# rssalessio/TZDDPC

Measured on NVIDIA B200. Metric: closed-loop TZDDPC steps/sec over batched scenarios, higher is better.
Workload: dtype f64

## Files before the change

### tzddpc_b200/csrc/tz_admm.cuh

```cuda
#pragma once
#include "tz_common.cuh"

namespace tz {

#ifndef TZ_SPO_MIN
#define TZ_SPO_MIN 16
#endif
template <int NZ_, int N2_, int NU_, int NL_, int G_, int NPAR_, int NAG_, int NCHK_, int MINB_>
struct Bucket {
  static constexpr int NZ = NZ_, N2 = N2_, NU = NU_, NL = NL_, G = G_, NPAR = NPAR_, NAG = NAG_, NCHK = NCHK_;
  static constexpr int MINB = MINB_;
  static constexpr int NCL = N2 + NU + NL;
  static constexpr int NC = NCL * G;
  static constexpr int NK = N2 * G;
  static constexpr int NCOL = 1 + 2 * NPAR + NAG;
  static constexpr int NCHL = (NCHK + G - 1) / G;
  static constexpr int TPB = 128;
  static constexpr int WPB = TPB / 32;
  static constexpr int SPW = 32 / G;
  static constexpr int TPO = (SPW >= TZ_SPO_MIN) ? 1 : TZ_SPO_MIN / SPW;
  static constexpr int SPO = SPW * TPO;
  static constexpr int HP = NPAR / 2;
  static constexpr int OM_V = 1, OM_P = 1 + NZ, NW = 1 + NZ + NPAR;
  static constexpr int OM_C = NW, OM_XP = NW + HP, KOM = NW + 2 * HP;
  static constexpr int PRE_ROWS = 4 * HP + G;
  static constexpr int NCOL2 = (NCOL + 1) / 2;
  static constexpr int NCOLP = 2 * NCOL2 + ((2 * NCOL2) % 8 == 0 ? 2 : 0);
  static_assert(NCL <= 32 && (G & (G - 1)) == 0 && G <= 32 && N2 >= 1 && NAG >= 1, "bad bucket");
};

template <class BK>
struct QpProg {
  double P[BK::NZ][BK::NZ];
  double A[BK::NC][BK::NZ];
  double l0[BK::NC], u0[BK::NC];
  double kink0[BK::NK], wabs[BK::NK];
  double R[BK::NC][BK::NCOLP];
  double Rs[BK::NC];
  double q0[BK::NZ];
  double Qp[BK::NZ][BK::NPAR];
  double Bt[BK::NAG][BK::NPAR];
  double gam[BK::NAG];
  double Rchk[BK::NCHK][BK::NCOLP];
  double chk_tol[BK::NCHK];
  double cc[BK::NCOL];
  double CC2[BK::NPAR][BK::NPAR];
  double D[BK::NZ];
  double Einv[BK::NC];
  double sing_inv[BK::NC];
  double cinv;
  int sing_var[BK::NC];
  int row_of_slot[BK::NC];
  int grp_order[BK::NC];
  int grp_new[BK::NC];
  double grp_sgn[BK::NC];
  int grp_first[BK::NC + 4];
  int ngrp;
// ... 671 lines not shown
```

### tzddpc_b200/csrc/tz_fast.cuh

```cuda
#pragma once
#include <cstdlib>

#include "tz_step.cuh"

namespace tz {

constexpr int kDeferTile = TZ_SPO_MIN;

constexpr int fast_ctas_per_sm(int tpb) { return tpb >= 512 ? 1 : 512 / tpb; }

template <class BK, int TPB, int NSLOT, int H = 1, bool PL = false>
__global__ void __launch_bounds__(TPB * H, fast_ctas_per_sm(TPB * H))
    fast_step_kernel(const QpProg<BK>* __restrict__ gpg, const Aux ax, const SolverParams sp, const StepArgs a,
                     const SetEntry* __restrict__ entries, const int32_t* __restrict__ tile_prog, const int slot_bytes) {
  constexpr int NZ = BK::NZ, NPAR = BK::NPAR, HP = BK::NPAR / 2, NCOL = BK::NCOL, NW = BK::NW, G = BK::G;
  static_assert(kDeferTile == 16 && BK::SPO == 16, "deferred tiles are the 16-scenario output tiles of step_kernel");
  static_assert(NSLOT <= 1 || TPB == 32, "two program slots: one warp per CTA");
  constexpr int OM_X = NW + HP, OM_NS = NW + 2 * HP;
  constexpr int QPB = (int)((sizeof(QpProg<BK>) + 15) & ~(size_t)15);
  extern __shared__ __align__(16) unsigned char smem_raw[];
  const int tix = threadIdx.x, tid = tix % TPB, hq = tix / TPB, lane = tix & 31;
  constexpr int NT = TPB * H;
  const int n = ax.n, m = ax.m, nv = ax.nv;
  const bool closed = a.x != nullptr;
  const int64_t LD = a.ld;
  const bool dense = a.ze1 != nullptr && !sp.tube_packed;
  double (*om)[TPB] = reinterpret_cast<double (*)[TPB]>(smem_raw + (NSLOT > 1 ? NSLOT : 1) * (size_t)slot_bytes);
  int* sflag = reinterpret_cast<int*>(&om[NW + 3 * HP][0]);
  const int n_tab = H > 1 ? ax.o_zrow : ax.n_dbl;
  auto stage = [&](unsigned char* slot, const void* pg_src, const double* tab_src) {
    const char* src = reinterpret_cast<const char*>(pg_src);
    char* dst = reinterpret_cast<char*>(slot);
    double* td = reinterpret_cast<double*>(slot + QPB);
    constexpr int NCH = (int)(sizeof(QpProg<BK>) / 16);
    for (int i = tix; i < NCH; i += NT) cp_async16(dst + 16 * i, src + 16 * i);
    if (tix == 0 && (sizeof(QpProg<BK>) % 16) != 0) cp_async8(dst + 16 * NCH, src + 16 * NCH);
    for (int i = tix; i < n_tab; i += NT) cp_async8(td + i, tab_src + i);
  };
  auto stage_plant = [&](unsigned char* slot) {
    double* td = reinterpret_cast<double*>(slot + QPB);
    if (closed && !PL) {
      for (int i = tix; i < n * n; i += NT) cp_async8(td + n_tab + i, a.A_true + i);
      for (int i = tix; i < n * m; i += NT) cp_async8(td + n_tab + n * n + i, a.B_true + i);
    }
  };
  pdl_trigger();
  unsigned char* my_slot = smem_raw;
  if constexpr (NSLOT == 0) {
    stage(smem_raw, gpg, ax.tab);
  } else {
    constexpr int TILES = TPB / kDeferTile;
    const int64_t last_tile = (a.S + kDeferTile - 1) / kDeferTile - 1;
    const int64_t t0 = (int64_t)blockIdx.x * TILES;
    const int j0 = tile_prog[t0 < last_tile ? t0 : last_tile];
    stage(smem_raw, entries[j0].pg, entries[j0].tab);
    if constexpr (NSLOT == 2) {
      const int j1 = tile_prog[t0 + 1 < last_tile ? t0 + 1 : last_tile];
      if (j1 != j0) {
        stage(smem_raw + slot_bytes, entries[j1].pg, entries[j1].tab);
        if (lane >= 16) my_slot = smem_raw + slot_bytes;
      }
    }
  }
  cp_async_commit();
  pdl_wait();
  stage_plant(smem_raw);
  if constexpr (NSLOT == 2) stage_plant(smem_raw + slot_bytes);
  cp_async_commit();
  double* tabd = reinterpret_cast<double*>(my_slot + QPB);
  bool staged = false;
  const QpProg<BK>& pg = *reinterpret_cast<const QpProg<BK>*>(my_slot);
  const double* sXB = tabd + ax.o_XB;
  const double* sCZ = tabd + ax.o_CZ;
  const double* sK = tabd + ax.o_K;
  const double* sA = tabd + n_tab;
  const double* sB = sA + n * n;
  const double2* tt = reinterpret_cast<const double2*>(tabd + ax.o_tt);
  const int* zs = reinterpret_cast<const int*>(tabd + ax.o_zrun);
  const bool zvec = dense && (reinterpret_cast<uintptr_t>(a.ze1) & 15u) == 0 && (a.ld & 1) == 0 && (a.S & 1) == 0 &&
                    (int64_t)(ax.n * (1 + ax.g1)) * a.ld * 8 < (int64_t)0x7fffffff;
  const int* zrow = reinterpret_cast<const int*>(tabd + ax.o_zrow);
  const int64_t nblk = (a.S + TPB - 1) / TPB;
  const unsigned long long* hint = reinterpret_cast<const unsigned long long*>(a.warm);
  unsigned long long* hint_w = reinterpret_cast<unsigned long long*>(a.warm);
  const unsigned half_mask = lane < 16 ? 0x0000ffffu : 0xffff0000u;
  const double* omc = &om[0][tid];

  for (int64_t blk = blockIdx.x; blk < nblk; blk += (NSLOT == 0 ? (int64_t)gridDim.x : nblk)) {
    const int64_t s = blk * TPB + tid;
    const bool live = s < a.S;
    const int64_t sc = live ? s : a.S - 1;
    bool emit = false, good = false;
    enum { kDefer = -2 };
    int status = kDefer;
    double omr[NW];
    double nrm2 = 0.0, cost = NAN;
    auto zero_runs = [&]() {
      double* base = a.ze1 + s;
#pragma unroll 1
      for (int r = 0; r < ax.n_zrun; ++r) {
        double* ptr = base + (int64_t)zs[2 * r] * LD;
#pragma unroll 4
        for (int c = zs[2 * r + 1]; c > 0; --c, ptr += LD) __stcs(ptr, 0.0);
      }
    };
    constexpr int CPR = TPB / 2;
    const int z_half = tid / CPR;
    const int64_t z_sv = blk * TPB + 2 * (tid % CPR);
    int z_pos = z_half * ax.n_zrow_half;
    const int z_stop = z_pos + ax.n_zrow_half;
    if (!(zvec && z_sv < a.S) || H > 1) z_pos = z_stop;
    char* const z_base = reinterpret_cast<char*>(a.ze1 + z_sv);
    const int ld8 = (int)(LD * 8);
    auto drip = [&](int budget) {
      int k = z_stop - z_pos;
      k = k < budget ? k : budget;
#pragma unroll 2
      for (; k > 0; k -= 4, z_pos += 4) {
        const int4 r = *reinterpret_cast<const int4*>(zrow + z_pos);
        const double2 z2 = make_double2(0.0, 0.0);
        __stcs(reinterpret_cast<double2*>(z_base + (int64_t)r.x * ld8), z2);
        __stcs(reinterpret_cast<double2*>(z_base + (int64_t)r.y * ld8), z2);
        __stcs(reinterpret_cast<double2*>(z_base + (int64_t)r.z * ld8), z2);
        __stcs(reinterpret_cast<double2*>(z_base + (int64_t)r.w * ld8), z2);
      }
    };
    const bool zero_first = H == 1 && dense && !zvec && (((tid >> 5) + (int)blk) & 1);
    if (hq == 0) {
    double w[2 * BK::NCOL2];
// ... 70 lines not shown
    if (__any_sync(0xffffffffu, status == kDefer && valid)) {
      const bool inf = singleton_infeasible2<BK>(pg, w);
      if (status == kDefer && valid && inf) status = TZ_STATUS_INFEASIBLE;
    }
    const unsigned dmask = __ballot_sync(0xffffffffu, live && status == kDefer);
    const bool deferred = (dmask & half_mask) != 0u;
    if (deferred && (lane & 15) == 0 && live) {
      const int slot = atomicAdd(a.defer, 1);
      if (slot >= 0 && slot < (a.S + kDeferTile - 1) / kDeferTile) a.defer_list[slot] = (int32_t)(s / kDeferTile);
    }
    emit = live && !deferred;
    good = status == TZ_STATUS_OK;
    drip(16);
    if (emit) {
#pragma unroll
      for (int g = 0; g < G; ++g) {
        unsigned long long wnext = 0ull;
        if (good) {
          wnext = code[g] | kCodeValid;
          if (fresh) hint_w[(int64_t)(G + g) * LD + s] = wnext;
        } else if (a.x_restart != nullptr) {
          const unsigned long long h0 = hint[(int64_t)(G + g) * LD + s];
          wnext = (h0 & kCodeValid) ? (h0 | kCodeFresh) : 0ull;
        }
        hint_w[(int64_t)g * LD + s] = wnext;
      }
      omr[0] = 1.0;
#pragma unroll
      for (int j = 0; j < NZ; ++j) omr[BK::OM_V + j] = (j < nv) ? (good ? pg.D[j] * res.x[j] : NAN) : 0.0;
#pragma unroll
      for (int j = 0; j < NPAR; ++j) omr[BK::OM_P + j] = w[1 + j];
      if (good) cost = fma(res.obj, pg.cinv, c0);
      else if (status == TZ_STATUS_INFEASIBLE) cost = INFINITY;
#pragma unroll
      for (int j = 0; j < NW; ++j) om[j][tid] = omr[j];
#pragma unroll 2
      for (int r = 0; r < n; ++r) {
        const double* row = sCZ + r * NW;
        double acc = 0.0;
#pragma unroll
        for (int j = 0; j < NW; ++j) acc = fma(row[j], omr[j], acc);
        om[BK::OM_C + r][tid] = acc;
      }
      drip(16);
    }
    if constexpr (H > 1) sflag[tid] = (emit ? 1 : 0) | (good ? 2 : 0);
    } else {
      if (!staged) {
        cp_async_wait<0>();
        __syncthreads();
        staged = true;
      }
      if (dense && live) {
        double* base = a.ze1 + s;
#pragma unroll 1
        for (int r = hq - 1; r < ax.n_zrun; r += H - 1) {
          double* ptr = base + (int64_t)zs[2 * r] * LD;
#pragma unroll 4
          for (int c = zs[2 * r + 1]; c > 0; --c, ptr += LD) __stcs(ptr, 0.0);
        }
      }
    }
    if constexpr (H > 1) {
      __syncthreads();
      if (hq > 0) {
        const int f = sflag[tid];
        emit = (f & 1) != 0;
        good = (f & 2) != 0;
        if (emit) {
#pragma unroll
          for (int j = 0; j < NW; ++j) omr[j] = omc[j * TPB];
        }
      }
    }
    if (emit) {
      if (a.ze1 != nullptr) {
        double* base = a.ze1 + s;
        if (sp.tube_packed) {
          double* ptr = base + (int64_t)hq * LD;
#pragma unroll 4
          for (int i = hq; i < ax.n_nz; i += H, ptr += H * LD) {
            const double2 e = tt[i];
            __stcs(ptr, e.x * omc[(int)(__double_as_longlong(e.y) & 0xffffffffll) * TPB]);
          }
        } else {
          if constexpr (H == 1) {
            if (!zero_first && !zvec) zero_runs();
          }
#pragma unroll 4
          for (int i = hq; i < ax.n_nz; i += H) {
            const double2 e = tt[i];
            const long long ie = __double_as_longlong(e.y);
            __stcs(base + (ie >> 32) * LD, e.x * omc[(int)(ie & 0xffffffffll) * TPB]);
          }
        }
      }
      double xb1[HP];
#pragma unroll
      for (int i = 0; i < HP; ++i) xb1[i] = 0.0;
      auto xb_row = [&](int i) {
        const double* row = sXB + i * NW;
        double acc = 0.0;
#pragma unroll
        for (int j = 0; j < NW; ++j) acc = fma(row[j], omr[j], acc);
        if (a.xbar_traj != nullptr) a.xbar_traj[(int64_t)i * LD + s] = acc;
        return acc;
      };
      if constexpr (H == 1) {
        if (a.xbar_traj != nullptr) {
#pragma unroll 2
          for (int i = 0; i < n; ++i) (void)xb_row(i);
        }
        drip(16);
        if (a.xbar_traj != nullptr || closed) {
#pragma unroll
          for (int k = 0; k < HP; ++k)
            if (k < n) xb1[k] = xb_row(n + k);
        }
        drip(16);
        if (a.xbar_traj != nullptr) {
#pragma unroll 2
          for (int i = 2 * n; i < (ax.N + 1) * n; ++i) (void)xb_row(i);
        }
      } else {
        if (hq == 0 && (a.xbar_traj != nullptr || closed)) {
#pragma unroll
          for (int k = 0; k < HP; ++k)
            if (k < n) xb1[k] = xb_row(n + k);
        }
        if (a.xbar_traj != nullptr && hq > 0) {
#pragma unroll 1
          for (int i = hq - 1; i < (ax.N + 1) * n; i += H - 1)
            if (i < n || i >= 2 * n) (void)xb_row(i);
        }
      }
      if (hq == 0) {
      if (a.v != nullptr)
        for (int j = 0; j < nv; ++j) a.v[(int64_t)j * LD + s] = omc[(BK::OM_V + j) * TPB];
      if (a.status) a.status[s] = status;
      if (a.iters) a.iters[s] = 0;
      if (a.cost) a.cost[s] = cost;
      if (closed) {
        double us[kMaxM];
#pragma unroll
        for (int j = 0; j < kMaxM; ++j) {
          double acc = 0.0;
          if (j < m) {
            acc = omr[BK::OM_V + (j < NZ ? j : 0)];
#pragma unroll
            for (int i = 0; i < HP; ++i)
              if (i < n) acc = fma(sK[j * n + i], omr[BK::OM_P + HP + i], acc);
            if (a.u_out) a.u_out[(int64_t)j * LD + s] = good ? acc : NAN;
          }
          us[j] = acc;
        }
        double xo[HP];
        cp_async_wait<0>();
#pragma unroll
        for (int i = 0; i < HP; ++i) xo[i] = (i < n) ? omc[(OM_X + i) * TPB] : 0.0;
#pragma unroll
        for (int i = 0; i < HP; ++i) {
          if (i < n) {
            double acc = a.noise ? omc[(OM_NS + i) * TPB] : 0.0;
            if constexpr (PL) {
              const double* ab = a.AB_true + (int64_t)i * (n + m) * LD + s;
#pragma unroll
              for (int k = 0; k < HP; ++k)
                if (k < n) acc = fma(ab[(int64_t)k * LD], xo[k], acc);
#pragma unroll
              for (int k = 0; k < kMaxM; ++k)
                if (k < m) acc = fma(ab[(int64_t)(n + k) * LD], us[k], acc);
// ... 135 lines not shown
```

### tzddpc_b200/csrc/tz_fused.cu

```cuda
#include "tz_step.cuh"
#include "tz_big.h"

namespace tz {

template <class BK>
int launch_fast(const TzProgram* p, const SolverParams& sp, const StepArgs& a, cudaStream_t st);
extern template int launch_fast<B0>(const TzProgram*, const SolverParams&, const StepArgs&, cudaStream_t);
template <class BK>
int launch_fast_set(const TzProgram* p0, const SolverParams& sp, const StepArgs& a, const SetEntry* entries, const int32_t* tile_prog,
                    int block, cudaStream_t st);
extern template int launch_fast_set<B0>(const TzProgram*, const SolverParams&, const StepArgs&, const SetEntry*, const int32_t*, int,
                                        cudaStream_t);
extern template int launch_bucket<B1>(const TzProgram*, const SolverParams&, const StepArgs&, cudaStream_t);
extern template int launch_bucket<B2>(const TzProgram*, const SolverParams&, const StepArgs&, cudaStream_t);
extern template int launch_bucket<B3>(const TzProgram*, const SolverParams&, const StepArgs&, cudaStream_t);
extern template int launch_bucket_set<B1>(const TzProgram*, const SetEntry*, int, int64_t, const SolverParams&, const StepArgs&, cudaStream_t);
extern template int launch_bucket_set<B2>(const TzProgram*, const SetEntry*, int, int64_t, const SolverParams&, const StepArgs&, cudaStream_t);
extern template int launch_bucket_set<B3>(const TzProgram*, const SetEntry*, int, int64_t, const SolverParams&, const StepArgs&, cudaStream_t);
extern template int launch_bucket_set_run<B1>(const TzProgram*, const SetEntry*, int, int64_t, const SolverParams&, const StepArgs&, cudaStream_t);
extern template int launch_bucket_set_run<B2>(const TzProgram*, const SetEntry*, int, int64_t, const SolverParams&, const StepArgs&, cudaStream_t);
extern template int launch_bucket_set_run<B3>(const TzProgram*, const SetEntry*, int, int64_t, const SolverParams&, const StepArgs&, cudaStream_t);

constexpr int64_t kHotMinBatch = 256;

struct RowClasses { int n2 = 0, nu = 0, nl = 0; };

static RowClasses classify(const TzProgramDesc& d, std::vector<int>* cls) {
  RowClasses rc;
  for (int i = 0; i < d.nc; ++i) {
    const bool lf = std::isfinite(d.l0[i]), uf = std::isfinite(d.u0[i]);
    int c = 0;
    if (d.wabs[i] > 0.0 || (lf && uf) || (!lf && !uf)) c = 0;
// ... 113 lines not shown
      g.grp_first[gi++] = t;
      for (size_t k = 0; k < mem.size(); ++k, ++t) {
        g.grp_order[t] = mem[k].first;
        g.grp_new[t] = k == 0 ? 1 : 0;
        g.grp_sgn[t] = mem[k].second;
      }
    }
    g.ngrp = gi;
    for (; gi < BK::NC + 4; ++gi) g.grp_first[gi] = t;
    for (; t < BK::NC; ++t) { g.grp_order[t] = 0; g.grp_new[t] = 0; g.grp_sgn[t] = 1.0; }
  }
  g.cinv = 1.0 / d.c;
  g.nz = nz; g.nc = nc; g.npar = npar; g.nag = nag; g.nchk = d.nchk;
  g.has_cc2 = 0;
  for (int a = 0; a < npar * npar; ++a) g.has_cc2 |= (d.CC2[a] != 0.0) ? 1 : 0;
}

}

using namespace tz;

struct HostImage {
  std::vector<unsigned char> packed, aux;
};

template <class BK>
static int create_bucket(const TzProgramDesc& d, TzProgram* p, int id, HostImage& img) {
  p->bucket = id;
  img.packed.assign(sizeof(QpProg<BK>), 0);
  pack<BK>(d, *reinterpret_cast<QpProg<BK>*>(img.packed.data()));
  p->NZ = BK::NZ;
  p->NC = BK::NC;
  p->G = BK::G;
  p->NW = BK::NW; p->OM_V = BK::OM_V; p->OM_P = BK::OM_P; p->OM_C = BK::OM_C; p->HP = BK::NPAR / 2;
  return TZ_OK;
}

static int use_big_path(const TzProgramDesc* d, TzProgram* p) {
  p->bucket = 4;
  p->NZ = d->nz; p->NC = d->nc; p->G = 32;
  p->nz = d->nz; p->nc = d->nc; p->n = d->n; p->m = d->m; p->N = d->horizon; p->nv = d->nv; p->g1 = d->g1; p->npar = d->npar;
  for (int e = 0; e < d->n * (1 + d->g1); ++e)
    if (d->ze1_ptr[e + 1] > d->ze1_ptr[e]) p->tube_ent.push_back(e);
  p->aux.n_nz = (int)p->tube_ent.size();
  p->aux.n = d->n; p->aux.m = d->m; p->aux.N = d->horizon; p->aux.nv = d->nv; p->aux.g1 = d->g1;
  return TZ_OK;
}

static int build_program_host(const TzProgramDesc* d, TzProgram* p, HostImage& img) {
  TZ_REQUIRE(d != nullptr, "null argument");
  TZ_REQUIRE(d->n >= 1 && d->n <= kMaxN && d->m >= 1 && d->m <= kMaxM, "dim_x must be 1..%d and dim_u 1..%d", kMaxN, kMaxM);
  TZ_REQUIRE(d->npar == 2 * d->n, "npar must be 2*dim_x");
  TZ_REQUIRE(d->nv == d->horizon * d->m && d->nv <= 16 && d->nz >= d->nv, "bad nv/nz");
  TZ_REQUIRE(d->nc >= 0 && d->na >= 0 && d->nchk >= 0 && d->g1 >= 0 && d->nterms >= 0 && d->nkink >= 0 && d->nkink <= d->nc,
             "negative size in the program descriptor");
  TZ_REQUIRE(d->ze1_ptr && d->ze1_ptr[0] == 0, "ze1_ptr[0] must be 0");
  for (int e = 0; e < d->n * (1 + d->g1); ++e)
    TZ_REQUIRE(d->ze1_ptr[e + 1] >= d->ze1_ptr[e], "ze1_ptr must be non-decreasing (entry %d)", e);
  TZ_REQUIRE(d->ze1_ptr[d->n * (1 + d->g1)] == d->nterms, "ze1_ptr[n(1+g1)] must equal nterms");
  int rc = TZ_ERANGE;
#define TZ_TRY(BK, ID) \
  if (rc == TZ_ERANGE && fits<BK>(*d)) rc = create_bucket<BK>(*d, p, ID, img);
  TZ_TRY(B0, 0) TZ_TRY(B1, 1) TZ_TRY(B2, 2) TZ_TRY(B3, 3)
#undef TZ_TRY
  if (rc == TZ_ERANGE && big_fits(*d)) return use_big_path(d, p);
  if (rc != TZ_OK) {
    if (rc == TZ_ERANGE) {
      const RowClasses c = classify(*d, nullptr);
      return fail(TZ_ERANGE, "program (nz=%d rows: %d two-sided, %d upper, %d lower; npar=%d general atoms=%d nchk=%d) "
                  "exceeds every compiled bucket", d->nz, c.n2, c.nu, c.nl, d->npar, general_atoms(*d, nullptr), d->nchk);
    }
    return rc;
  }
  p->nz = d->nz; p->nc = d->nc; p->n = d->n; p->m = d->m; p->N = d->horizon; p->nv = d->nv; p->g1 = d->g1; p->npar = d->npar;
  const int n = d->n, nwc = 1 + d->nv + d->npar, ld1 = 1 + d->g1, nent = n * ld1, NW = p->NW;
  auto omidx = [&](int j) {
    if (j == 0) return 0;
    if (j <= d->nv) return p->OM_V + (j - 1);
    const int k = j - 1 - d->nv;
    return k < n ? p->OM_P + k : p->OM_P + p->HP + (k - n);
  };
  const int nrows = (d->horizon + 1) * n;
  std::vector<double> XB((size_t)nrows * NW, 0.0), CZ((size_t)n * NW, 0.0), coef;
  std::vector<int32_t> ent, idx;
  for (int i = 0; i < nrows; ++i)
    for (int j = 0; j < nwc; ++j) XB[(size_t)i * NW + omidx(j)] = d->XB[(size_t)i * nwc + j];
  for (int e = 0; e < nent; ++e) {
    const int t0 = d->ze1_ptr[e], t1 = d->ze1_ptr[e + 1];
    for (int t = t0; t < t1; ++t)
      if (d->ze1_idx[t] < 0 || d->ze1_idx[t] >= nwc) return fail(TZ_EINVAL, "ze1_idx[%d] out of range", t);
    const int r = e / ld1, j = e % ld1;
    if (j == 0) {
      for (int t = t0; t < t1; ++t) CZ[(size_t)r * NW + omidx(d->ze1_idx[t])] += d->ze1_val[t];
      ent.push_back(e); idx.push_back(p->OM_C + r); coef.push_back(1.0);
    } else if (t1 - t0 == 1) {
      ent.push_back(e); idx.push_back(omidx(d->ze1_idx[t0])); coef.push_back(d->ze1_val[t0]);
    } else if (t1 - t0 > 1) {
      return fail(TZ_EINVAL, "generator entry %d of Ze[1] has %d terms: only single-term generator entries are supported "
                  "(boxed M_K / M_Delta)", e, t1 - t0);
    }
  }
  std::vector<int32_t> zstart, zlen;
  {
    int next = 0;
    for (size_t i = 0; i <= ent.size(); ++i) {
      const int stop = i < ent.size() ? ent[i] : nent;
      if (stop > next) { zstart.push_back(next); zlen.push_back(stop - next); }
      next = stop + 1;
    }
  }
  const size_t nXB = XB.size(), nCZ = CZ.size(), nK = (size_t)d->m * n, nco = coef.size();
  const size_t o_tt = (nXB + nCZ + nK + nco + 1) & ~(size_t)1;
  const size_t o_zrun = o_tt + 2 * nco;
  int zrun_split = 0;
  {
    int total = 0, acc = 0;
    for (int v : zlen) total += v;
    while (zrun_split < (int)zlen.size() && 2 * acc < total) acc += zlen[zrun_split++];
  }
  std::vector<int32_t> zrow;
  int n_zrow_half = 0;
  {
    std::vector<int32_t> all;
    for (size_t i = 0; i < zstart.size(); ++i)
      for (int c = 0; c < zlen[i]; ++c) all.push_back(zstart[i] + c);
    const size_t h0 = (all.size() + 1) / 2, h1 = all.size() - h0;
    n_zrow_half = (int)((std::max(h0, h1) + 3) & ~(size_t)3);
    if (h1 == 0) n_zrow_half = all.empty() ? 0 : n_zrow_half;
    zrow.assign((size_t)2 * n_zrow_half, 0);
    for (int half = 0; half < 2 && !all.empty(); ++half) {
      const size_t b = half == 0 ? 0 : h0, cnt = half == 0 ? h0 : h1;
      for (int k = 0; k < n_zrow_half; ++k) {
        const size_t src = cnt == 0 ? h0 - 1 : b + std::min((size_t)k, cnt - 1);
        zrow[(size_t)half * n_zrow_half + k] = all[src];
      }
    }
  }
  const size_t o_zrow = (o_zrun + zstart.size() + 1) & ~(size_t)1;
  const size_t ndbl = o_zrow + (size_t)n_zrow_half, nint = ent.size() + idx.size();
  const size_t smem_tab = (ndbl + (size_t)n * n + (size_t)n * d->m) * sizeof(double) + nint * sizeof(int32_t);
  if (smem_tab > kMaxTabBytes) {
    if (big_fits(*d)) {
      *p = TzProgram();
      img = HostImage();
      return use_big_path(d, p);
    }
    return fail(TZ_ERANGE, "program tables need %zu bytes of shared memory (limit %d)", smem_tab, kMaxTabBytes);
  }
  std::vector<unsigned char>& host = img.aux;
  host.assign(ndbl * sizeof(double) + nint * sizeof(int32_t) + 16, 0);
  double* hd = reinterpret_cast<double*>(host.data());
  std::memcpy(hd, XB.data(), nXB * sizeof(double));
  std::memcpy(hd + nXB, CZ.data(), nCZ * sizeof(double));
  std::memcpy(hd + nXB + nCZ, d->K, nK * sizeof(double));
  if (nco) std::memcpy(hd + nXB + nCZ + nK, coef.data(), nco * sizeof(double));
  int32_t* hi = reinterpret_cast<int32_t*>(hd + ndbl);
  if (!ent.empty()) std::memcpy(hi, ent.data(), ent.size() * sizeof(int32_t));
  if (!idx.empty()) std::memcpy(hi + ent.size(), idx.data(), idx.size() * sizeof(int32_t));
  for (size_t i = 0; i < nco; ++i) {
    hd[o_tt + 2 * i] = coef[i];
    const long long bits = (long long)(uint32_t)idx[i] | ((long long)ent[i] << 32);
    std::memcpy(&hd[o_tt + 2 * i + 1], &bits, sizeof(bits));
  }
  for (size_t i = 0; i < zstart.size(); ++i) {
    const int32_t pr[2] = {zstart[i], zlen[i]};
    std::memcpy(&hd[o_zrun + i], pr, sizeof(pr));
  }
  if (!zrow.empty()) std::memcpy(&hd[o_zrow], zrow.data(), zrow.size() * sizeof(int32_t));
  Aux& ax = p->aux;
  ax.tab = nullptr;
  ax.n_dbl = (int)ndbl; ax.n_int = (int)nint;
  ax.o_XB = 0; ax.o_CZ = (int)nXB; ax.o_K = (int)(nXB + nCZ); ax.o_coef = (int)(nXB + nCZ + nK);
  ax.o_ent = 0; ax.o_idx = (int)ent.size();
  ax.o_tt = (int)o_tt; ax.o_zrun = (int)o_zrun; ax.n_zrun = (int)zstart.size();
  ax.zrun_split = zrun_split;
  ax.o_zrow = (int)o_zrow; ax.n_zrow_half = n_zrow_half;
  ax.n_nz = (int)ent.size();
  p->tube_ent = ent;
  ax.n = n; ax.m = d->m; ax.N = d->horizon; ax.nv = d->nv; ax.g1 = d->g1;
  p->smem_tab = (smem_tab + 15) & ~(size_t)15;
  return TZ_OK;
}

static int device_info(TzProgram* p) {
  int dev = 0;
  TZ_CUDA(cudaGetDevice(&dev));
  p->device = dev;
  TZ_CUDA(cudaDeviceGetAttribute(&p->num_sms, cudaDevAttrMultiProcessorCount, dev));
  return TZ_OK;
}

extern "C" int tz_program_create(const TzProgramDesc* d, TzProgram** out) {
  TZ_REQUIRE(d && out, "null argument");
  TzProgram* p = new (std::nothrow) TzProgram();
  if (!p) return fail(TZ_ENOMEM, "out of host memory");
  HostImage img;
  int rc = build_program_host(d, p, img);
  if (rc == TZ_OK) rc = device_info(p);
  if (rc == TZ_OK && p->bucket == 4) rc = big_create(*d, &p->big);
  if (rc != TZ_OK) {
    delete p;
    return rc;
  }
  if (p->bucket == 4) {
    *out = p;
    return TZ_OK;
  }
// ... 274 lines not shown
extern "C" int tz_program_tube_pattern(const TzProgram* p, int32_t* entries_host, int32_t cap) {
  if (!p) return fail(TZ_EINVAL, "null program");
  const int nnz = p->aux.n_nz;
  if (entries_host) {
    TZ_REQUIRE(cap >= nnz, "tube pattern needs %d entries (cap %d)", nnz, cap);
    std::memcpy(entries_host, p->tube_ent.data(), (size_t)nnz * sizeof(int32_t));
  }
  return nnz;
}

struct TzProgramSet {
  std::vector<const TzProgram*> progs;
  std::vector<int64_t> begin;
  tz::SetEntry* entries_dev = nullptr;
  int32_t* tile_prog_dev = nullptr;
  int block = 16;
  int64_t max_scen = 0, total_tiles = 0;
};

extern "C" int tz_program_set_create(const TzProgram* const* progs, int32_t nprog, const int64_t* begin, TzProgramSet** out) {
  TZ_REQUIRE(progs && begin && out && nprog >= 1, "null argument / empty set");
  const TzProgram* p0 = progs[0];
  TZ_REQUIRE(p0 != nullptr, "null program 0");
  TZ_REQUIRE(begin[0] == 0, "begin[0] must be 0");
  std::vector<tz::SetEntry> ent((size_t)nprog);
  int64_t mx = 0, tiles = 0;
  for (int j = 0; j < nprog; ++j) {
    const TzProgram* p = progs[j];
    TZ_REQUIRE(p != nullptr, "null program %d", j);
    const Aux &a = p->aux, &b = p0->aux;
    TZ_REQUIRE(p->bucket != 4, "programs of the generic large-program path cannot be combined into a set");
    TZ_REQUIRE(p->bucket == p0->bucket && p->smem_tab == p0->smem_tab && a.n_dbl == b.n_dbl && a.n_int == b.n_int &&
               a.o_XB == b.o_XB && a.o_CZ == b.o_CZ && a.o_K == b.o_K && a.o_coef == b.o_coef && a.o_ent == b.o_ent &&
               a.o_idx == b.o_idx && a.o_tt == b.o_tt && a.o_zrun == b.o_zrun && a.n_zrun == b.n_zrun && a.zrun_split == b.zrun_split && a.o_zrow == b.o_zrow && a.n_zrow_half == b.n_zrow_half && a.n_nz == b.n_nz && a.n == b.n && a.m == b.m && a.N == b.N && a.nv == b.nv && a.g1 == b.g1,
               "program %d does not have the structure of program 0 (bucket / table sizes differ)", j);
    TZ_REQUIRE(p->tube_ent == p0->tube_ent, "program %d: Ze[1] has a different sparsity pattern than program 0", j);
    const int64_t cnt = begin[j + 1] - begin[j];
    TZ_REQUIRE(cnt >= 0, "begin[] must be non-decreasing");
    TZ_REQUIRE(begin[j] % 16 == 0, "begin[%d] = %lld: the scenarios of a program must start on a multiple of 16", j,
               (long long)begin[j]);
    ent[j] = tz::SetEntry{p->packed_dev, a.tab, begin[j], begin[j + 1], tiles};
    tiles += (cnt + TZ_SPO_MIN - 1) / TZ_SPO_MIN;
    if (cnt > mx) mx = cnt;
  }
  TzProgramSet* s = new (std::nothrow) TzProgramSet();
  if (!s) return fail(TZ_ENOMEM, "out of host memory");
  s->progs.assign(progs, progs + nprog);
  s->begin.assign(begin, begin + nprog + 1);
  s->max_scen = mx;
  s->total_tiles = tiles;
  std::vector<int32_t> tile_prog((size_t)((begin[nprog] + TZ_SPO_MIN - 1) / TZ_SPO_MIN) + 1, nprog - 1);
  s->block = 128;
  for (int j = 0; j < nprog; ++j) {
    for (int64_t t = begin[j] / TZ_SPO_MIN; t < (begin[j + 1] + TZ_SPO_MIN - 1) / TZ_SPO_MIN; ++t) tile_prog[(size_t)t] = j;
    if (begin[j + 1] > begin[j])
      while (s->block > 16 && begin[j] % s->block != 0) s->block /= 2;
  }
  cudaError_t err = cudaMalloc(&s->entries_dev, ent.size() * sizeof(tz::SetEntry));
  if (err == cudaSuccess) err = cudaMemcpy(s->entries_dev, ent.data(), ent.size() * sizeof(tz::SetEntry), cudaMemcpyHostToDevice);
  if (err == cudaSuccess) err = cudaMalloc(&s->tile_prog_dev, tile_prog.size() * sizeof(int32_t));
  if (err == cudaSuccess)
    err = cudaMemcpy(s->tile_prog_dev, tile_prog.data(), tile_prog.size() * sizeof(int32_t), cudaMemcpyHostToDevice);
  if (err != cudaSuccess) {
    if (s->entries_dev) cudaFree(s->entries_dev);
    if (s->tile_prog_dev) cudaFree(s->tile_prog_dev);
    delete s;
    return fail(TZ_ECUDA, "program set upload: %s", cudaGetErrorString(err));
// ... 273 lines not shown
```

### tzddpc_b200/csrc/tz_step.cuh

```cuda
#pragma once
#include <atomic>
#include <cmath>
#include <new>
#include <type_traits>
#include <vector>

#include "tz_admm.cuh"
#include "tz_cert2.cuh"
#include "tz_param.cuh"

#define TZ_LIKELY(x) __builtin_expect(!!(x), 1)
#define TZ_UNLIKELY(x) __builtin_expect(!!(x), 0)

namespace tz {

struct Aux {
  const double* tab;
  int n_dbl, n_int;
  int o_XB, o_CZ, o_K, o_coef;
  int o_ent, o_idx;
  int o_tt;
  int o_zrun, n_zrun;
  int zrun_split;
  int o_zrow, n_zrow_half;
  int n_nz;
  int n, m, N, nv, g1;
};

struct StepArgs {
  int64_t S;
  int64_t ld;
  int vec2;
  const double* xbar0;
  const double* e0;
  double* x;
  double* xbar;
  double* e;
  const double* noise;
  const double* x_restart;
  const double* A_true;
  const double* B_true;
  double* cost;
  double* v;
  double* xbar_traj;
  double* ze1;
  double* u_out;
  int32_t* status;
  int32_t* iters;
  double* warm;
  double* stats;
  const double* q_in;
  const double* l_in;
  const double* u_in;
  double* z_out;
// ... 142 lines not shown
#pragma unroll
  for (int t = 0; t < W; ++t) {
    stt[t] = wb.status[sc0 + t];
    olive[t] = stt[t] >= 0;
    ogood[t] = stt[t] == TZ_STATUS_OK || stt[t] == TZ_STATUS_MAXITER;
    any_live = any_live || olive[t];
    all_good = all_good && ogood[t];
  }
  auto om = [&](int j) { return vld(&wb.om[j][sc0], vt); };
  if (a.ze1 && packed) {
    if (any_live) {
      double* base = a.ze1 + so;
      const double* coef = tabd + ax.o_coef;
      const int* idx = tabi + ax.o_idx;
#pragma unroll 4
      for (int i = slice; i < ax.n_nz; i += NSL) vstcs(base + (int64_t)i * LD, vmul(coef[i], om(idx[i])));
    }
  } else if (a.ze1) {
    if (any_live && !zero_done) zero_fill<BK, W>(ax, a, tile, lane);
    __syncwarp();
    if (any_live) {
      double* base = a.ze1 + so;
      const double* coef = tabd + ax.o_coef;
      const int* ent = tabi + ax.o_ent;
      const int* idx = tabi + ax.o_idx;
#pragma unroll 4
      for (int i = slice; i < ax.n_nz; i += NSL) vstcs(base + (int64_t)ent[i] * LD, vmul(coef[i], om(idx[i])));
    }
  }
  if (any_live) {
    if (a.xbar_traj) {
      const int nrows = (ax.N + 1) * n;
      for (int i = slice; i < nrows; i += NSL) {
        const double* row = sXB + i * NW;
        V acc = vzero(vt);
#pragma unroll
        for (int j = 0; j < NW; ++j) acc = vfma(row[j], om(j), acc);
        vst(a.xbar_traj + (int64_t)i * LD + so, acc);
      }
    }
    if (a.v)
      for (int j = slice; j < nv; j += NSL) vst(a.v + (int64_t)j * LD + so, om(BK::OM_V + j));
    if (slice == 0) {
#pragma unroll
      for (int t = 0; t < W; ++t) {
        if (olive[t]) {
          if (a.status) a.status[so + t] = stt[t];
          if (a.iters) a.iters[so + t] = wb.iters[sc0 + t];
          if (a.cost) a.cost[so + t] = wb.cost[sc0 + t];
        }
      }
    }
  }
  if (a.x != nullptr) {
    const double* sK = tabd + ax.o_K;
    const double* sA = tabd + ax.n_dbl;
    const double* sB = sA + n * n;
    if (any_live) {
      V us[kMaxM];
#pragma unroll
      for (int j = 0; j < kMaxM; ++j) {
        V acc = vzero(vt);
        if (j < m) {
          acc = om(BK::OM_V + j);
          for (int i = 0; i < n; ++i) acc = vfma(sK[j * n + i], om(BK::OM_P + BK::NPAR / 2 + i), acc);
          if (a.u_out && slice == 0) vst(a.u_out + (int64_t)j * LD + so, vsel(ogood, acc, NAN));
        }
        us[j] = acc;
      }
      for (int i = slice; i < n; i += NSL) {
        V acc = a.noise ? vld(&pre[3 * n + i][sc0], vt) : vzero(vt);
        if constexpr (PL) {
          const double* ab = a.AB_true + (int64_t)i * (n + m) * LD + so;
          for (int k = 0; k < n; ++k) acc = vfma2(vld(ab + (int64_t)k * LD, vt), vld(&pre[2 * n + k][sc0], vt), acc);
#pragma unroll
          for (int k = 0; k < kMaxM; ++k)
            if (k < m) acc = vfma2(vld(ab + (int64_t)(n + k) * LD, vt), us[k], acc);
        } else {
          for (int k = 0; k < n; ++k) acc = vfma(sA[i * n + k], vld(&pre[2 * n + k][sc0], vt), acc);
#pragma unroll
          for (int k = 0; k < kMaxM; ++k)
            if (k < m) acc = vfma(sB[i * m + k], us[k], acc);
        }
        const double* row = sXB + (n + i) * NW;
        V xb1 = vzero(vt);
#pragma unroll
        for (int j = 0; j < NW; ++j) xb1 = vfma(row[j], om(j), xb1);
        V en = vsub(acc, xb1);
        if (TZ_UNLIKELY(!all_good)) {
          const V xo = vld(&pre[2 * n + i][sc0], vt);
          const V xbo = om(BK::OM_P + i), eo = om(BK::OM_P + BK::NPAR / 2 + i);
          const V xr = a.x_restart ? vld(a.x_restart + (int64_t)i * LD + so, vt) : xo;
          double xa[W], ba[W], ea[W];
#pragma unroll
          for (int t = 0; t < W; ++t) {
            xa[t] = ogood[t] ? vget(acc, t) : vget(xr, t);
            ba[t] = ogood[t] ? vget(xb1, t) : (a.x_restart ? vget(xr, t) : vget(xbo, t));
            ea[t] = ogood[t] ? vget(en, t) : (a.x_restart ? 0.0 : vget(eo, t));
          }
          if constexpr (W == 1) { acc = V{xa[0]}; xb1 = V{ba[0]}; en = V{ea[0]}; }
          else { acc = V{xa[0], xa[1]}; xb1 = V{ba[0], ba[1]}; en = V{ea[0], ea[1]}; }
        }
        vst(&wb.om[BK::OM_XP + i][sc0], acc);
        vst(a.x + (int64_t)i * LD + so, acc);
        if (a.x_hist != nullptr) vst(a.x_hist + (int64_t)i * LD + so, acc);
        if (a.xbar_hist != nullptr) vst(a.xbar_hist + (int64_t)i * LD + so, xb1);
        if (a.e_hist != nullptr) vst(a.e_hist + (int64_t)i * LD + so, en);
        vst(a.xbar + (int64_t)i * LD + so, xb1);
        vst(a.e + (int64_t)i * LD + so, en);
      }
    }
    if (a.stats != nullptr) {
      __syncwarp();
      if (slice == 0) {
#pragma unroll
        for (int t = 0; t < W; ++t) {
          if (olive[t]) {
// ... 289 lines not shown
#pragma unroll
    for (int k = 0; k < N2; ++k) {
      double axv = 0.0;
#pragma unroll
      for (int j = 0; j < NZ; ++j) axv = fma(qp.Aa[k][j], st.x[j], axv);
      kcost = fma(qp.wk[k * G], fabs(axv * inv_alpha - qp.kink[k]), kcost);
    }
    kcost = gsum<G>(kcost);
    double cost = NAN;
    if (good) {
      double acc = kcost;
#pragma unroll
      for (int j = 0; j < NZ; ++j) {
        double px = 0.0;
#pragma unroll
        for (int b = 0; b < NZ; ++b) px = fma(qp.P[j][b], st.x[b], px);
        acc = fma(0.5 * px + qp.q[j], st.x[j], acc);
      }
      cost = fma(acc, pg.cinv, c0);
      if (NZ == 2 && hint_ok) cost = fma(hint_obj, pg.cinv, c0);
    } else if (live && status == TZ_STATUS_INFEASIBLE) {
      cost = INFINITY;
    }
    if (g == 0) {
      wb.om[0][col] = 1.0;
#pragma unroll
      for (int j = 0; j < NZ; ++j) wb.om[BK::OM_V + j][col] = (j < nv) ? (good ? pg.D[j] * st.x[j] : NAN) : 0.0;
      wb.cost[col] = cost;
      wb.status[col] = live ? status : -1;
      wb.iters[col] = iters;
    }
    __syncwarp();
    for (int r = g; r < n; r += G) {
      const double* row = sCZ + r * NW;
      double acc = 0.0;
#pragma unroll
      for (int j = 0; j < NW; ++j) acc = fma(row[j], wb.om[j][col], acc);
      wb.om[BK::OM_C + r][col] = acc;
    }
   }
    if (explicit_qp) continue;
    __syncwarp();
    if (TZ_LIKELY(a.vec2)) output_phase<BK, 2, PL>(wb, pre, ax, a, tabd, tabi, otile, lane, zslot < BK::TPO, sp.tube_packed != 0);
    else output_phase<BK, 1, PL>(wb, pre, ax, a, tabd, tabi, otile, lane, zslot < BK::TPO, sp.tube_packed != 0);
    __syncwarp();
  }
  if (a.stats != nullptr && a.x != nullptr) {
    __syncwarp();
    if (lane < TZ_NSTATS) {
      double v_ = 0.0;
#pragma unroll
      for (int c = 0; c < BK::SPO; ++c) v_ += wb.stacc[lane][c];
      if (v_ != 0.0) atomicAdd(a.stats + lane, v_);
    }
  }
}

__device__ __forceinline__ StepArgs step_block(const StepArgs& a, const Aux& ax, const int64_t tube_rows, const int k) {
  const int64_t LD = a.ld;
  StepArgs ak = a;
  if (ak.noise) ak.noise += (int64_t)k * ax.n * LD;
  if (ak.cost) ak.cost += (int64_t)k * LD;
  if (ak.v) ak.v += (int64_t)k * ax.nv * LD;
  if (ak.xbar_traj) ak.xbar_traj += (int64_t)k * (ax.N + 1) * ax.n * LD;
  if (ak.ze1) ak.ze1 += (int64_t)k * tube_rows * LD;
  if (ak.u_out) ak.u_out += (int64_t)k * ax.m * LD;
  ak.status += (int64_t)k * LD;
// ... 173 lines not shown
    Aux ax = ax0;
    ax.tab = en.tab;
    StepArgs a = shift_args<PL>(a0, en.begin, en.end - en.begin);
    a.list_mode = 0;
    const bool stage = staged != j;
    if (stage && staged >= 0) __syncthreads();
    staged = j;
    const int64_t tl = t - en.begin / BK::SPO;
    run_program<BK, PL>(smem_raw, reinterpret_cast<const QpProg<BK>*>(en.pg), ax, sp, a, tl, BK::WPB, tl + 1, (unsigned)(t % 1024), stage);
  }
  __syncthreads();
  if (threadIdx.x == 0) {
    const int tk = atomicAdd(a0.defer + 1, 1);
    if (tk == (int)gridDim.x - 1) { a0.defer[0] = 0; a0.defer[1] = 0; }
  }
}

using B0 = Bucket<2, 1, 3, 3, 4, 10, 2, 12, 3>;
using B1 = Bucket<4, 2, 4, 4, 8, 16, 8, 32, 3>;
using B2 = Bucket<8, 3, 5, 5, 8, 16, 24, 32, 2>;
using B3 = Bucket<12, 1, 4, 4, 8, 16, 24, 32, 1>;

}

namespace tz { struct BigProgram; }

struct TzProgram {
  int bucket = -1;
  void* packed_dev = nullptr;
  void* aux_dev = nullptr;
  tz::Aux aux{};
  int nz = 0, nc = 0, n = 0, m = 0, N = 0, nv = 0, g1 = 0, npar = 0;
  int NZ = 0, NC = 0, G = 0;
  int NW = 0, OM_V = 0, OM_P = 0, OM_C = 0, HP = 0;
  std::vector<int32_t> tube_ent;
  size_t smem_tab = 0;
  int num_sms = 148;
  int device = -1;
  bool owns_device = true;
  tz::BigProgram* big = nullptr;
};

template <class K>
int ensure_dynamic_smem(K kernel, int bytes, int device, std::atomic<unsigned long long>& done) {
  const unsigned long long bit = 1ull << (device & 63);
  if (device >= 0 && device < 64 && (done.load(std::memory_order_relaxed) & bit)) return TZ_OK;
  TZ_CUDA(cudaFuncSetAttribute(kernel, cudaFuncAttributeMaxDynamicSharedMemorySize, bytes));
  if (device >= 0 && device < 64) done.fetch_or(bit, std::memory_order_relaxed);
  return TZ_OK;
}

constexpr int kMaxTabBytes = 24 * 1024;


namespace tz {

template <class BK, auto kernel, class... Args>
int launch_step(const TzProgram* p, unsigned grid, cudaStream_t st, int64_t S, Args... args) {
  static std::atomic<unsigned long long> configured{0ull};
  if (const int rc = ensure_dynamic_smem(kernel, (int)(sizeof(Smem<BK>) + kMaxTabBytes), p->device, configured)) return rc;
  TZ_CUDA(launch_kernel(kernel, grid, BK::TPB, sizeof(Smem<BK>) + p->smem_tab, st, pdl_enabled(S), args...));
  return TZ_OK;
}

template <class BK>
int launch_bucket(const TzProgram* p, const SolverParams& sp, const StepArgs& a, cudaStream_t st) {
  const int64_t ntiles = (a.S + BK::SPO - 1) / BK::SPO;
// ... 46 lines not shown
```

Before: 1.054 billion.

## Sort tube entries by source column and keep omega in registers for emit

Host packing now sorts the Ze[1] tube entries by their omega source index and builds a per-source column pointer table. In the H==1 fast kernel this lets the emit loop read each omega value from registers instead of storing omega to shared memory and gathering it back. XB and CZ rows are padded to an even width so the dot products can use double2 loads, and the CZ products are held in registers. The risk is extra register pressure and an inner loop with variable trip count per source, plus added table space.

```diff
diff --git a/tzddpc_b200/csrc/tz_admm.cuh b/tzddpc_b200/csrc/tz_admm.cuh
--- a/tzddpc_b200/csrc/tz_admm.cuh
+++ b/tzddpc_b200/csrc/tz_admm.cuh
@@ -23,6 +23,7 @@
   static constexpr int HP = NPAR / 2;
   static constexpr int OM_V = 1, OM_P = 1 + NZ, NW = 1 + NZ + NPAR;
   static constexpr int OM_C = NW, OM_XP = NW + HP, KOM = NW + 2 * HP;
+  static constexpr int NWP = (NW + 1) & ~1;
   static constexpr int PRE_ROWS = 4 * HP + G;
   static constexpr int NCOL2 = (NCOL + 1) / 2;
   static constexpr int NCOLP = 2 * NCOL2 + ((2 * NCOL2) % 8 == 0 ? 2 : 0);
diff --git a/tzddpc_b200/csrc/tz_fast.cuh b/tzddpc_b200/csrc/tz_fast.cuh
--- a/tzddpc_b200/csrc/tz_fast.cuh
+++ b/tzddpc_b200/csrc/tz_fast.cuh
@@ -13,7 +13,7 @@
 __global__ void __launch_bounds__(TPB * H, fast_ctas_per_sm(TPB * H))
     fast_step_kernel(const QpProg<BK>* __restrict__ gpg, const Aux ax, const SolverParams sp, const StepArgs a,
                      const SetEntry* __restrict__ entries, const int32_t* __restrict__ tile_prog, const int slot_bytes) {
-  constexpr int NZ = BK::NZ, NPAR = BK::NPAR, HP = BK::NPAR / 2, NCOL = BK::NCOL, NW = BK::NW, G = BK::G;
+  constexpr int NZ = BK::NZ, NPAR = BK::NPAR, HP = BK::NPAR / 2, NCOL = BK::NCOL, NW = BK::NW, NWP = BK::NWP, G = BK::G;
   static_assert(kDeferTile == 16 && BK::SPO == 16, "deferred tiles are the 16-scenario output tiles of step_kernel");
   static_assert(NSLOT <= 1 || TPB == 32, "two program slots: one warp per CTA");
   constexpr int OM_X = NW + HP, OM_NS = NW + 2 * HP;
@@ -76,6 +76,7 @@
   const double* sA = tabd + n_tab;
   const double* sB = sA + n * n;
   const double2* tt = reinterpret_cast<const double2*>(tabd + ax.o_tt);
+  const int* tcol = reinterpret_cast<const int*>(tabd + ax.o_tcol);
   const int* zs = reinterpret_cast<const int*>(tabd + ax.o_zrun);
   const bool zvec = dense && (reinterpret_cast<uintptr_t>(a.ze1) & 15u) == 0 && (a.ld & 1) == 0 && (a.S & 1) == 0 &&
                     (int64_t)(ax.n * (1 + ax.g1)) * a.ld * 8 < (int64_t)0x7fffffff;
@@ -93,8 +94,19 @@
     bool emit = false, good = false;
     enum { kDefer = -2 };
     int status = kDefer;
-    double omr[NW];
+    double omr[NW], cz[HP];
     double nrm2 = 0.0, cost = NAN;
+    auto dot_om = [&](const double* row) {
+      const double2* r2 = reinterpret_cast<const double2*>(row);
+      double acc = 0.0;
+#pragma unroll
+      for (int j = 0; j < NWP / 2; ++j) {
+        const double2 c = r2[j];
+        acc = fma(c.x, omr[2 * j], acc);
+        if (2 * j + 1 < NW) acc = fma(c.y, omr[2 * j + 1], acc);
+      }
+      return acc;
+    };
     auto zero_runs = [&]() {
       double* base = a.ze1 + s;
 #pragma unroll 1
@@ -231,15 +243,14 @@
       for (int j = 0; j < NPAR; ++j) omr[BK::OM_P + j] = w[1 + j];
       if (good) cost = fma(res.obj, pg.cinv, c0);
       else if (status == TZ_STATUS_INFEASIBLE) cost = INFINITY;
-#pragma unroll
-      for (int j = 0; j < NW; ++j) om[j][tid] = omr[j];
+      if constexpr (H == 1) {
+#pragma unroll
+        for (int r = 0; r < HP; ++r) cz[r] = r < n ? dot_om(sCZ + r * NWP) : 0.0;
+      } else {
+#pragma unroll
+        for (int j = 0; j < NW; ++j) om[j][tid] = omr[j];
 #pragma unroll 2
-      for (int r = 0; r < n; ++r) {
-        const double* row = sCZ + r * NW;
-        double acc = 0.0;
-#pragma unroll
-        for (int j = 0; j < NW; ++j) acc = fma(row[j], omr[j], acc);
-        om[BK::OM_C + r][tid] = acc;
+        for (int r = 0; r < n; ++r) om[BK::OM_C + r][tid] = dot_om(sCZ + r * NWP);
       }
       drip(16);
     }
@@ -275,33 +286,31 @@
     if (emit) {
       if (a.ze1 != nullptr) {
         double* base = a.ze1 + s;
-        if (sp.tube_packed) {
-          double* ptr = base + (int64_t)hq * LD;
-#pragma unroll 4
-          for (int i = hq; i < ax.n_nz; i += H, ptr += H * LD) {
-            const double2 e = tt[i];
-            __stcs(ptr, e.x * omc[(int)(__double_as_longlong(e.y) & 0xffffffffll) * TPB]);
+        if constexpr (H == 1) {
+          if (!sp.tube_packed && !zero_first && !zvec) zero_runs();
+        }
+        const int row_shift = sp.tube_packed ? 32 : 0;
+        auto emit_source = [&](int j, double val) {
+#pragma unroll 1
+          for (int k = tcol[j] + hq; k < tcol[j + 1]; k += H) {
+            const double2 e = tt[k];
+            const int row = (int)(__double_as_longlong(e.y) >> row_shift);
+            __stcs(base + (int64_t)row * LD, e.x * val);
           }
+        };
+        if constexpr (H == 1) {
+#pragma unroll
+          for (int j = 0; j < NW + HP; ++j) emit_source(j, j < NW ? omr[j] : cz[j - NW]);
         } else {
-          if constexpr (H == 1) {
-            if (!zero_first && !zvec) zero_runs();
-          }
-#pragma unroll 4
-          for (int i = hq; i < ax.n_nz; i += H) {
-            const double2 e = tt[i];
-            const long long ie = __double_as_longlong(e.y);
-            __stcs(base + (ie >> 32) * LD, e.x * omc[(int)(ie & 0xffffffffll) * TPB]);
-          }
+#pragma unroll 1
+          for (int j = 0; j < NW + HP; ++j) emit_source(j, omc[j * TPB]);
         }
       }
       double xb1[HP];
 #pragma unroll
       for (int i = 0; i < HP; ++i) xb1[i] = 0.0;
       auto xb_row = [&](int i) {
-        const double* row = sXB + i * NW;
-        double acc = 0.0;
-#pragma unroll
-        for (int j = 0; j < NW; ++j) acc = fma(row[j], omr[j], acc);
+        const double acc = dot_om(sXB + i * NWP);
         if (a.xbar_traj != nullptr) a.xbar_traj[(int64_t)i * LD + s] = acc;
         return acc;
       };
@@ -335,7 +344,9 @@
       }
       if (hq == 0) {
       if (a.v != nullptr)
-        for (int j = 0; j < nv; ++j) a.v[(int64_t)j * LD + s] = omc[(BK::OM_V + j) * TPB];
+#pragma unroll
+        for (int j = 0; j < NZ; ++j)
+          if (j < nv) a.v[(int64_t)j * LD + s] = omr[BK::OM_V + j];
       if (a.status) a.status[s] = status;
       if (a.iters) a.iters[s] = 0;
       if (a.cost) a.cost[s] = cost;
diff --git a/tzddpc_b200/csrc/tz_fused.cu b/tzddpc_b200/csrc/tz_fused.cu
--- a/tzddpc_b200/csrc/tz_fused.cu
+++ b/tzddpc_b200/csrc/tz_fused.cu
@@ -1,3 +1,5 @@
+#include <algorithm>
+
 #include "tz_step.cuh"
 #include "tz_big.h"
 
@@ -177,7 +179,7 @@
   p->NZ = BK::NZ;
   p->NC = BK::NC;
   p->G = BK::G;
-  p->NW = BK::NW; p->OM_V = BK::OM_V; p->OM_P = BK::OM_P; p->OM_C = BK::OM_C; p->HP = BK::NPAR / 2;
+  p->NW = BK::NW; p->NWP = BK::NWP; p->OM_V = BK::OM_V; p->OM_P = BK::OM_P; p->OM_C = BK::OM_C; p->HP = BK::NPAR / 2;
   return TZ_OK;
 }
 
@@ -218,7 +220,7 @@
     return rc;
   }
   p->nz = d->nz; p->nc = d->nc; p->n = d->n; p->m = d->m; p->N = d->horizon; p->nv = d->nv; p->g1 = d->g1; p->npar = d->npar;
-  const int n = d->n, nwc = 1 + d->nv + d->npar, ld1 = 1 + d->g1, nent = n * ld1, NW = p->NW;
+  const int n = d->n, nwc = 1 + d->nv + d->npar, ld1 = 1 + d->g1, nent = n * ld1, NWP = p->NWP;
   auto omidx = [&](int j) {
     if (j == 0) return 0;
     if (j <= d->nv) return p->OM_V + (j - 1);
@@ -226,17 +228,17 @@
     return k < n ? p->OM_P + k : p->OM_P + p->HP + (k - n);
   };
   const int nrows = (d->horizon + 1) * n;
-  std::vector<double> XB((size_t)nrows * NW, 0.0), CZ((size_t)n * NW, 0.0), coef;
+  std::vector<double> XB((size_t)nrows * NWP, 0.0), CZ((size_t)n * NWP, 0.0), coef;
   std::vector<int32_t> ent, idx;
   for (int i = 0; i < nrows; ++i)
-    for (int j = 0; j < nwc; ++j) XB[(size_t)i * NW + omidx(j)] = d->XB[(size_t)i * nwc + j];
+    for (int j = 0; j < nwc; ++j) XB[(size_t)i * NWP + omidx(j)] = d->XB[(size_t)i * nwc + j];
   for (int e = 0; e < nent; ++e) {
     const int t0 = d->ze1_ptr[e], t1 = d->ze1_ptr[e + 1];
     for (int t = t0; t < t1; ++t)
       if (d->ze1_idx[t] < 0 || d->ze1_idx[t] >= nwc) return fail(TZ_EINVAL, "ze1_idx[%d] out of range", t);
     const int r = e / ld1, j = e % ld1;
     if (j == 0) {
-      for (int t = t0; t < t1; ++t) CZ[(size_t)r * NW + omidx(d->ze1_idx[t])] += d->ze1_val[t];
+      for (int t = t0; t < t1; ++t) CZ[(size_t)r * NWP + omidx(d->ze1_idx[t])] += d->ze1_val[t];
       ent.push_back(e); idx.push_back(p->OM_C + r); coef.push_back(1.0);
     } else if (t1 - t0 == 1) {
       ent.push_back(e); idx.push_back(omidx(d->ze1_idx[t0])); coef.push_back(d->ze1_val[t0]);
@@ -255,8 +257,15 @@
     }
   }
   const size_t nXB = XB.size(), nCZ = CZ.size(), nK = (size_t)d->m * n, nco = coef.size();
+  const int nsrc = p->NW + p->HP;
+  std::vector<int32_t> tord(nco), tcol((size_t)nsrc + 1, 0);
+  for (size_t i = 0; i < nco; ++i) tord[i] = (int32_t)i;
+  std::stable_sort(tord.begin(), tord.end(), [&](int32_t x, int32_t y) { return idx[x] < idx[y]; });
+  for (size_t i = 0; i < nco; ++i) ++tcol[(size_t)idx[i] + 1];
+  for (int j = 0; j < nsrc; ++j) tcol[(size_t)j + 1] += tcol[(size_t)j];
   const size_t o_tt = (nXB + nCZ + nK + nco + 1) & ~(size_t)1;
-  const size_t o_zrun = o_tt + 2 * nco;
+  const size_t o_tcol = o_tt + 2 * nco;
+  const size_t o_zrun = o_tcol + (tcol.size() + 1) / 2;
   int zrun_split = 0;
   {
     int total = 0, acc = 0;
@@ -302,11 +311,13 @@
   int32_t* hi = reinterpret_cast<int32_t*>(hd + ndbl);
   if (!ent.empty()) std::memcpy(hi, ent.data(), ent.size() * sizeof(int32_t));
   if (!idx.empty()) std::memcpy(hi + ent.size(), idx.data(), idx.size() * sizeof(int32_t));
-  for (size_t i = 0; i < nco; ++i) {
-    hd[o_tt + 2 * i] = coef[i];
-    const long long bits = (long long)(uint32_t)idx[i] | ((long long)ent[i] << 32);
-    std::memcpy(&hd[o_tt + 2 * i + 1], &bits, sizeof(bits));
-  }
+  for (size_t k = 0; k < nco; ++k) {
+    const int32_t i = tord[k];
+    hd[o_tt + 2 * k] = coef[(size_t)i];
+    const long long bits = (long long)(uint32_t)ent[(size_t)i] | ((long long)i << 32);
+    std::memcpy(&hd[o_tt + 2 * k + 1], &bits, sizeof(bits));
+  }
+  std::memcpy(&hd[o_tcol], tcol.data(), tcol.size() * sizeof(int32_t));
   for (size_t i = 0; i < zstart.size(); ++i) {
     const int32_t pr[2] = {zstart[i], zlen[i]};
     std::memcpy(&hd[o_zrun + i], pr, sizeof(pr));
@@ -317,7 +328,7 @@
   ax.n_dbl = (int)ndbl; ax.n_int = (int)nint;
   ax.o_XB = 0; ax.o_CZ = (int)nXB; ax.o_K = (int)(nXB + nCZ); ax.o_coef = (int)(nXB + nCZ + nK);
   ax.o_ent = 0; ax.o_idx = (int)ent.size();
-  ax.o_tt = (int)o_tt; ax.o_zrun = (int)o_zrun; ax.n_zrun = (int)zstart.size();
+  ax.o_tt = (int)o_tt; ax.o_tcol = (int)o_tcol; ax.o_zrun = (int)o_zrun; ax.n_zrun = (int)zstart.size();
   ax.zrun_split = zrun_split;
   ax.o_zrow = (int)o_zrow; ax.n_zrow_half = n_zrow_half;
   ax.n_nz = (int)ent.size();
@@ -658,7 +669,7 @@
     TZ_REQUIRE(p->bucket != 4, "programs of the generic large-program path cannot be combined into a set");
     TZ_REQUIRE(p->bucket == p0->bucket && p->smem_tab == p0->smem_tab && a.n_dbl == b.n_dbl && a.n_int == b.n_int &&
                a.o_XB == b.o_XB && a.o_CZ == b.o_CZ && a.o_K == b.o_K && a.o_coef == b.o_coef && a.o_ent == b.o_ent &&
-               a.o_idx == b.o_idx && a.o_tt == b.o_tt && a.o_zrun == b.o_zrun && a.n_zrun == b.n_zrun && a.zrun_split == b.zrun_split && a.o_zrow == b.o_zrow && a.n_zrow_half == b.n_zrow_half && a.n_nz == b.n_nz && a.n == b.n && a.m == b.m && a.N == b.N && a.nv == b.nv && a.g1 == b.g1,
+               a.o_idx == b.o_idx && a.o_tt == b.o_tt && a.o_tcol == b.o_tcol && a.o_zrun == b.o_zrun && a.n_zrun == b.n_zrun && a.zrun_split == b.zrun_split && a.o_zrow == b.o_zrow && a.n_zrow_half == b.n_zrow_half && a.n_nz == b.n_nz && a.n == b.n && a.m == b.m && a.N == b.N && a.nv == b.nv && a.g1 == b.g1,
                "program %d does not have the structure of program 0 (bucket / table sizes differ)", j);
     TZ_REQUIRE(p->tube_ent == p0->tube_ent, "program %d: Ze[1] has a different sparsity pattern than program 0", j);
     const int64_t cnt = begin[j + 1] - begin[j];
diff --git a/tzddpc_b200/csrc/tz_step.cuh b/tzddpc_b200/csrc/tz_step.cuh
--- a/tzddpc_b200/csrc/tz_step.cuh
+++ b/tzddpc_b200/csrc/tz_step.cuh
@@ -20,6 +20,7 @@
   int o_XB, o_CZ, o_K, o_coef;
   int o_ent, o_idx;
   int o_tt;
+  int o_tcol;
   int o_zrun, n_zrun;
   int zrun_split;
   int o_zrow, n_zrow_half;
@@ -228,7 +229,7 @@
     if (a.xbar_traj) {
       const int nrows = (ax.N + 1) * n;
       for (int i = slice; i < nrows; i += NSL) {
-        const double* row = sXB + i * NW;
+        const double* row = sXB + i * BK::NWP;
         V acc = vzero(vt);
 #pragma unroll
         for (int j = 0; j < NW; ++j) acc = vfma(row[j], om(j), acc);
@@ -278,7 +279,7 @@
           for (int k = 0; k < kMaxM; ++k)
             if (k < m) acc = vfma(sB[i * m + k], us[k], acc);
         }
-        const double* row = sXB + (n + i) * NW;
+        const double* row = sXB + (n + i) * BK::NWP;
         V xb1 = vzero(vt);
 #pragma unroll
         for (int j = 0; j < NW; ++j) xb1 = vfma(row[j], om(j), xb1);
@@ -634,7 +635,7 @@
     }
     __syncwarp();
     for (int r = g; r < n; r += G) {
-      const double* row = sCZ + r * NW;
+      const double* row = sCZ + r * BK::NWP;
       double acc = 0.0;
 #pragma unroll
       for (int j = 0; j < NW; ++j) acc = fma(row[j], wb.om[j][col], acc);
@@ -874,7 +875,7 @@
   tz::Aux aux{};
   int nz = 0, nc = 0, n = 0, m = 0, N = 0, nv = 0, g1 = 0, npar = 0;
   int NZ = 0, NC = 0, G = 0;
-  int NW = 0, OM_V = 0, OM_P = 0, OM_C = 0, HP = 0;
+  int NW = 0, NWP = 0, OM_V = 0, OM_P = 0, OM_C = 0, HP = 0;
   std::vector<int32_t> tube_ent;
   size_t smem_tab = 0;
   int num_sms = 148;
```

Result: no change. 1.062 billion, median of 6 (+0.7%).
